# OpenSpaceAI/Nesie

Hardware: AMD Instinct MI355X
Metric: ScanNet scenes/sec (fwd+bwd, 40k pts, bs=8) (higher is better)
Workload: dtype f32; 1 GPU; Nesie-VoteNet supervised pretrain step (nesie-votenet-scannet-pretrain-10%): fwd+bwd+AdamW, 40000 pts/scene, fp32, random-init weights; scenes_per_gpu=8, global_batch=8, parallelism=single, world_size=1, hip_graph=True, deterministic_backward=True, index_chain_pipelined=True, forward_cu_budget=232, forward_cu_budget_from_the_head_on=248, grad_allreduce_bytes=10561936, resident_input_scenes=0

## Files before the change

include/nesie_ops.h:

```cpp
#ifndef NESIE_OPS_H_
#define NESIE_OPS_H_

#include <stddef.h>
#include <stdint.h>

#ifdef __cplusplus
extern "C" {
#endif

typedef enum {
  NESIE_OK = 0,
  NESIE_ERR_INVALID_ARG = 1,
  NESIE_ERR_UNSUPPORTED = 2,
  NESIE_ERR_LAUNCH = 3
} nesie_status;

int nesie_abi_version(void);
const char *nesie_last_error(void);

int nesie_set_distance_form(int form);
int nesie_get_distance_form(void);
int nesie_set_cu_count(int n);
int nesie_get_cu_count(void);

// ... 5 lines not shown
                                     int *idx, void *workspace, size_t workspace_bytes,
                                     void *stream);

int nesie_furthest_point_sampling_with_dist_wrapper(int b, int n, int m,
                                                    const float *dist,
                                                    float *temp, int *idx,
                                                    void *stream);

int nesie_ball_query_wrapper(int b, int n, int m, float min_radius,
                             float max_radius, int nsample,
                             const float *new_xyz, const float *xyz, int *idx,
                             void *stream);

int nesie_fps_leaves_index(int b, int n);
int nesie_ball_query_indexed(int b, int n, int m, float min_radius, float max_radius,
                             int nsample, const float *new_xyz, const void *fps_workspace,
                             size_t workspace_bytes, int *idx, void *stream);

int nesie_knn_wrapper(int b, int n, int m, int nsample, const float *xyz,
                      const float *new_xyz, int *idx, float *dist2, void *stream);

int nesie_group_points_forward(int b, int c, int n, int npoints, int nsample,
                               const float *points, const int *idx, float *out,
                               void *stream);

int nesie_group_points_backward(int b, int c, int n, int npoints, int nsample,
                                const float *grad_out, const int *idx,
                                float *grad_points, void *stream);

int nesie_query_and_group_forward(int b, int c, int n, int npoints, int nsample,
                                  const float *xyz, const float *centres,
                                  const float *features, const int *idx, float radius,
                                  float *out, void *stream);
int nesie_query_and_group_backward(int b, int c, int n, int npoints, int nsample,
                                   const float *grad_out, const int *idx, float *grad_features,
                                   void *stream);
int nesie_inverted_index(int b, int n, long long e_total, const int *idx, int *order,
                         int *sources, int *scratch, void *stream);
int nesie_group_points_backward_csr(int b, int c, int n, int npoints, int nsample,
                                    const float *grad_out, const int *order, const int *sources,
                                    float *grad_points, void *stream);
int nesie_query_and_group_backward_csr(int b, int c, int n, int npoints, int nsample,
                                       const float *grad_out, const int *order,
                                       const int *sources, float *grad_features, void *stream);

int nesie_vote_finish_forward(int b, int c, int n, int normalise, const float *raw,
                              const float *seed_points, const float *seed_feats, float *vote_points,
                              float *vote_feats, float *inv_norm, void *stream);
int nesie_vote_finish_backward(int b, int c, int n, int normalise, const float *g_feats,
                               const float *g_points, const float *vote_feats, const float *inv_norm,
                               float *d_raw, void *stream);

int nesie_gather_rows3(int b, int n, int m, const float *xyz, const int *sample, float *centres,
                       void *stream);
int nesie_query_and_group_backward_xyz(int b, int c, int n, int npoints, int nsample, float radius,
                                       const float *grad_out, const int *order,
                                       const int *sources, const int *sample,
                                       const float *d_centres, float *d_xyz, void *stream);

int nesie_three_interpolate_grad_csr(int b, int c, int n, int m, const float *grad_out,
                                     long long grad_out_bstride, const float *weight, const int *order,
                                     const int *sources, float *grad_points, void *stream);

int nesie_gather_points_wrapper(int b, int c, int n, int npoints,
                                const float *points, const int *idx, float *out,
                                void *stream);

int nesie_gather_points_grad_wrapper(int b, int c, int n, int npoints,
                                     const float *grad_out, const int *idx,
                                     float *grad_points, void *stream);

int nesie_three_nn_wrapper(int b, int n, int m, const float *unknown,
                           const float *known, float *dist2, int *idx,
                           void *stream);

int nesie_three_interpolate_wrapper(int b, int c, int m, int n,
                                    const float *points, const int *idx,
                                    const float *weight, float *out,
                                    void *stream);

int nesie_grid_taps(int b, int kprop, int gp, int m, const float *centre, const float *size,
                    const float *heading, const float *mult, const float *plane,
                    const float *known, int *idx, float *weight, float *rel, void *stream);

int nesie_blend_conv_forward(int b, int c, int m, int n, const float *table, int pitch,
                             int seg_off, const int *idx, const float *weight,
                             const float *rel, const float *wx, float *out, int segs,
                             int seg_len, int c_total, int c_offset,
                             float *stat_partial , void *stream);
int nesie_blend_conv_runs(int n, int segs);
int nesie_blend_conv_backward(int b, int c, int m, int n, const float *dy, int pitch, int seg_off, const int *idx, const float *weight,
                              const float *rel, float *d_table, float *d_wx, int segs,
                              int seg_len, void *stream);
int nesie_blend_conv_backward_bn(int b, int c, int m, int n, const float *da, const float *z,
                                 const float *bnb, int pitch, int seg_off, const int *idx,
                                 const float *weight, const float *rel, float *d_table,
                                 float *d_wx, int segs, int seg_len, void *stream);

size_t nesie_blend_conv_backward_workspace_bytes(int b, int c, int n, int segs);
int nesie_blend_conv_backward_staged(int b, int c, int m, int n, const float *dy, const float *z,
                                     const float *bnb, int pitch, int seg_off, const int *idx,
                                     const float *weight, const float *rel, float *d_table,
                                     float *d_wx, int segs, int seg_len, void *workspace,
                                     size_t workspace_bytes, void *stream);
size_t nesie_blend_conv_backward_any_workspace_bytes(int b, int c, int m, int n, int segs);
int nesie_blend_conv_backward_any(int b, int c, int m, int n, const float *dy, const float *z,
                                  const float *bnb, int pitch, int seg_off, const int *idx,
                                  const float *weight, const float *rel, float *d_table,
                                  float *d_wx, int segs, int seg_len, void *workspace,
                                  size_t workspace_bytes, void *stream);
int nesie_channel_sum(int nb, int ng, int c, long long p, const float *x, long long x_bstride,
                      float *out, void *stream);

int nesie_pw_bnb_coef(int channels, int nslots, double count, const float *part,
                      const float *z_coef, const float *gamma, float *bnb, float *dgamma,
                      float *dbeta, void *stream);

int nesie_three_interpolate_grad_wrapper(int b, int c, int n, int m,
                                         const float *grad_out, const int *idx,
                                         const float *weight,
                                         float *grad_points, void *stream);

int nesie_sort_vertices_forward(int b, int n, int m, const float *vertices,
                                const uint8_t *mask, const int *num_valid,
                                int *idx, void *stream);

int nesie_points_in_boxes_batch(int b, int boxes_num, int pts_num,
                                const float *boxes, const float *pts, int *out,
                                void *stream);

int nesie_points_in_boxes_gpu(int b, int boxes_num, int pts_num, const float *boxes,
                              const float *pts, int *out, void *stream);

int nesie_roiaware_pool3d_sizes(int boxes_num, int pts_num, int channels, int out_x, int out_y,
                                int out_z, int max_pts_each_voxel, long long *out);
int nesie_roiaware_pool3d_forward(int boxes_num, int pts_num, int channels,
                                  int max_pts_each_voxel, int out_x, int out_y, int out_z,
                                  const float *rois, const float *pts, const float *pts_feature,
                                  int *argmax, int *pts_idx_of_voxels, float *pooled_features,
                                  int *pts_voxel, int pool_method, void *stream);
int nesie_roiaware_pool3d_backward(int boxes_num, int pts_num, int out_x, int out_y, int out_z,
                                   int channels, int max_pts_each_voxel,
                                   const int *pts_idx_of_voxels, const int *argmax,
                                   const int *pts_voxel, const float *grad_out, float *grad_in,
                                   int pool_method, void *stream);

int nesie_group_max_pool_forward(long long rows, int nsample, const float *x, float *out,
                                 uint8_t *argmax, void *stream);
int nesie_group_max_pool_backward(long long rows, int nsample, const float *grad_out,
                                  const uint8_t *argmax, float *grad_x, void *stream);
int nesie_group_max_pool_backward_add(long long rows, int nsample, const float *grad_out,
                                      const uint8_t *argmax, float *grad_x, void *stream);

int nesie_lhs_nms_samecls(int b, int k, const float *boxes, float thr, uint8_t *keep,
                          void *stream);

int nesie_iou3d_forward(int n, const float *box1, const float *box2, float *iou, float *jac,
                        void *stream);

int nesie_giou3d_forward(int n, const float *box1, const float *box2, int kind, int enclosing,
                         float *loss, float *iou, float *jac, void *stream);

int nesie_aa_iou3d_paired_forward(int n, const float *box1, const float *box2, int mode, float eps,
                                  float *out, float *jac1, float *jac2, void *stream);
int nesie_aa_iou3d_matrix_forward(int b, int m, int n, const float *box1, const float *box2,
                                  int mode, float eps, float *out, void *stream);
// ... 222 lines not shown
```

nesie_amd/csrc/interpolate.hip:

```cpp
#include "common.h"
#include <math.h>

namespace nesie {

constexpr int NN_BLOCK = 256;
constexpr int NN_TILE = 1024;

template <int FORM>
__global__ __launch_bounds__(NN_BLOCK) void three_nn_kernel(
    int n, int m, const float *__restrict__ unknown, const float *__restrict__ known,
    float *__restrict__ dist2, int *__restrict__ idx) {
  __shared__ float4 kk[NN_TILE];
  const int bi = blockIdx.y;
  const int q = blockIdx.x * NN_BLOCK + threadIdx.x;
  const bool live = q < n;
  unknown += (size_t)bi * n * 3;
  known += (size_t)bi * m * 3;
  const int qq = live ? q : n - 1;
  const float ux = unknown[qq * 3 + 0], uy = unknown[qq * 3 + 1], uz = unknown[qq * 3 + 2];
  float b1 = INFINITY, b2 = INFINITY, b3 = INFINITY;
  int i1 = 0, i2 = 0, i3 = 0;
  for (int t0 = 0; t0 < m; t0 += NN_TILE) {
    const int tn = m - t0 < NN_TILE ? m - t0 : NN_TILE;
    __syncthreads();
    for (int i = threadIdx.x; i < tn; i += NN_BLOCK)
      kk[i] = make_float4(known[(t0 + i) * 3 + 0], known[(t0 + i) * 3 + 1],
                          known[(t0 + i) * 3 + 2], 0.f);
    __syncthreads();
#pragma unroll 4
    for (int i = 0; i < tn; ++i) {
      const float4 kp = kk[i];
      const float d = sqdist_form<FORM>(ux - kp.x, uy - kp.y, uz - kp.z);
      if (d < b3) {
        const int k = t0 + i;
        if (d < b1) {
          b3 = b2; i3 = i2; b2 = b1; i2 = i1; b1 = d; i1 = k;
        } else if (d < b2) {
          b3 = b2; i3 = i2; b2 = d; i2 = k;
        } else {
          b3 = d; i3 = k;
        }
      }
    }
  }
  if (live) {
    float *od = dist2 + ((size_t)bi * n + q) * 3;
    int *oi = idx + ((size_t)bi * n + q) * 3;
    od[0] = b1; od[1] = b2; od[2] = b3;
    oi[0] = i1; oi[1] = i2; oi[2] = i3;
  }
}

template <int FORM>
__global__ __launch_bounds__(NN_BLOCK) void grid_taps_kernel(
    int kprop, int gp, int m, const float *__restrict__ centre, const float *__restrict__ size,
    const float *__restrict__ heading, const float *__restrict__ mult,
    const float *__restrict__ plane, const float *__restrict__ known, int *__restrict__ idx,
    float *__restrict__ weight, float *__restrict__ rel) {
  __shared__ float4 kk[NN_TILE];
  const int bi = blockIdx.y;
  const int n = kprop * gp;
  const int q = blockIdx.x * NN_BLOCK + threadIdx.x;
  const bool live = q < n;
  const int qq = live ? q : n - 1;
  const int k = qq / gp, g = qq - k * gp;
  const float *c3 = centre + ((size_t)bi * kprop + k) * 3;
  const float *s3 = size + ((size_t)bi * kprop + k) * 3;
  const float cx = c3[0], cy = c3[1], cz = c3[2];
  float l[3];
#pragma unroll
  for (int d = 0; d < 3; ++d) {
    const float f = __fmul_rn(mult[g * 3 + d], s3[d]) / 2.f;
    l[d] = __fadd_rn(f, __fmul_rn(f, plane[g * 3 + d]));
  }
  const float h = heading[(size_t)bi * kprop + k];
  const float ch = cosf(h), sh = sinf(h);
  const float ux = __fadd_rn(__fadd_rn(__fmul_rn(l[0], ch), __fmul_rn(l[1], sh)), cx);
  const float uy = __fadd_rn(__fadd_rn(__fmul_rn(l[0], -sh), __fmul_rn(l[1], ch)), cy);
  const float uz = __fadd_rn(l[2], cz);
  known += (size_t)bi * m * 3;
  float b1 = INFINITY, b2 = INFINITY, b3 = INFINITY;
  int i1 = 0, i2 = 0, i3 = 0;
  for (int t0 = 0; t0 < m; t0 += NN_TILE) {
    const int tn = m - t0 < NN_TILE ? m - t0 : NN_TILE;
    __syncthreads();
    for (int i = threadIdx.x; i < tn; i += NN_BLOCK)
      kk[i] = make_float4(known[(t0 + i) * 3 + 0], known[(t0 + i) * 3 + 1],
                          known[(t0 + i) * 3 + 2], 0.f);
    __syncthreads();
#pragma unroll 4
    for (int i = 0; i < tn; ++i) {
      const float4 kp = kk[i];
      const float d = sqdist_form<FORM>(ux - kp.x, uy - kp.y, uz - kp.z);
      if (d < b3) {
        const int kidx = t0 + i;
        if (d < b1) {
          b3 = b2; i3 = i2; b2 = b1; i2 = i1; b1 = d; i1 = kidx;
        } else if (d < b2) {
          b3 = b2; i3 = i2; b2 = d; i2 = kidx;
        } else {
          b3 = d; i3 = kidx;
        }
      }
    }
  }
  if (live) {
    const size_t o = ((size_t)bi * n + q) * 3;
    const float w1 = 1.f / __fadd_rn(sqrtf(b1), 1e-8f), w2 = 1.f / __fadd_rn(sqrtf(b2), 1e-8f),
                w3 = 1.f / __fadd_rn(sqrtf(b3), 1e-8f);
    const float ws = __fadd_rn(__fadd_rn(w1, w2), w3);
    idx[o] = i1; idx[o + 1] = i2; idx[o + 2] = i3;
    weight[o] = w1 / ws; weight[o + 1] = w2 / ws; weight[o + 2] = w3 / ws;
    rel[o] = ux - cx; rel[o + 1] = uy - cy; rel[o + 2] = uz - cz;
  }
}

constexpr int TI_BLOCK = 256;
constexpr int TI_CH = 8;

__global__ __launch_bounds__(TI_BLOCK) void three_interpolate_kernel(
    int c, int m, int n, const float *__restrict__ points, const int *__restrict__ idx,
    const float *__restrict__ weight, float *__restrict__ out) {
  const int p = blockIdx.x * TI_BLOCK + threadIdx.x;
  const int c0 = blockIdx.y * TI_CH;
  const int bi = blockIdx.z;
  if (p >= n) return;
  const int *ix = idx + ((size_t)bi * n + p) * 3;
  const float *w = weight + ((size_t)bi * n + p) * 3;
  int j0 = ix[0], j1 = ix[1], j2 = ix[2];
  j0 = j0 < 0 ? 0 : (j0 >= m ? m - 1 : j0);
  j1 = j1 < 0 ? 0 : (j1 >= m ? m - 1 : j1);
  j2 = j2 < 0 ? 0 : (j2 >= m ? m - 1 : j2);
  const float w0 = w[0], w1 = w[1], w2 = w[2];
  const int cend = c - c0 < TI_CH ? c - c0 : TI_CH;
#pragma unroll
  for (int i = 0; i < TI_CH; ++i) {
    if (i < cend) {
      const float *src = points + ((size_t)bi * c + c0 + i) * m;
      float r = __fadd_rn(__fadd_rn(__fmul_rn(w0, src[j0]), __fmul_rn(w1, src[j1])),
                          __fmul_rn(w2, src[j2]));
      out[((size_t)bi * c + c0 + i) * n + p] = r;
    }
  }
}

constexpr int TS_Q = 64;
constexpr int BF_LD = TS_Q + 1;
typedef float bf_f2 __attribute__((ext_vector_type(2)));
constexpr int BF_NQ = 8;

template <int CPT, bool WX, bool STAT>
__global__ __launch_bounds__(256) void blend_fwd_kernel(
    int c, int cb, int m, int n, int segs, int seg_len, int c_total, int c_offset, int pitch,
    int seg_off, const float *__restrict__ table, const int *__restrict__ idx,
    const float *__restrict__ weight, const float *__restrict__ rel,
    const float *__restrict__ wx, float *__restrict__ out, float *__restrict__ stat_partial,
    int nb) {
#pragma clang fp contract(off)
  constexpr int CW = CPT * 64;
  extern __shared__ float bf_lds[];
  float *tile = bf_lds;
  float *red = bf_lds + CW * BF_LD;
  const int bi = blockIdx.x % nb;
  const int q0 = (blockIdx.x / nb) * TS_Q;
  const int c0 = cb + blockIdx.y * CW;
  const int per_seg = n / segs;
  const int sg = q0 / per_seg, r0 = q0 - sg * per_seg;
  const int lane = threadIdx.x & 63, wv = threadIdx.x >> 6;
  int pj[3];
  float pw[3], pr[3];
  {
    const int r = r0 + wv * 16 + (lane & 15);
    const int k = r / seg_len, g = r - k * seg_len;
    const size_t p = (size_t)bi * n + (size_t)(k * segs + sg) * seg_len + g;
#pragma unroll
    for (int t = 0; t < 3; ++t) {
      const int j = idx[p * 3 + t];
      pj[t] = j < 0 ? 0 : (j >= m ? m - 1 : j);
      pw[t] = weight[p * 3 + t];
      pr[t] = WX ? rel[p * 3 + t] : 0.f;
    }
  }
  const float *feat = table + (size_t)bi * m * pitch + (size_t)sg * seg_off + c0;
  const unsigned voff = (unsigned)(lane * CPT * 4);
  float x[CPT][3] = {};
  if (WX) {
    __builtin_memcpy(&x[0][0], wx + ((size_t)sg * c + c0 + lane * CPT) * 3, sizeof(x));
  }
  constexpr int CP2 = CPT / 2;
  bf_f2 s2[CP2 ? CP2 : 1], q2[CP2 ? CP2 : 1];
  float s1 = 0.f, q1 = 0.f;
#pragma unroll
  for (int e = 0; e < CP2; ++e) s2[e] = q2[e] = bf_f2{0.f, 0.f};
#pragma unroll
  for (int i0 = 0; i0 < 16; i0 += BF_NQ) {
    float a[BF_NQ][3][CPT];
// ... 414 lines not shown
      int u = 0;
      for (; u + 3 < cntj; u += 4) {
        Row v[4];
#pragma unroll
        for (int k = 0; k < 4; ++k) v[k].load(base + (size_t)__builtin_amdgcn_readlane(myslot, u + k) * C);
#pragma unroll
        for (int k = 0; k < 4; ++k)
#pragma unroll
          for (int e = 0; e < CPT; ++e) acc.v[e] += v[k].v[e];
      }
      for (; u < cntj; ++u) {
        Row v;
        v.load(base + (size_t)__builtin_amdgcn_readlane(myslot, u) * C);
#pragma unroll
        for (int e = 0; e < CPT; ++e) acc.v[e] += v.v[e];
      }
    }
  }
  acc.store(d_table + ((size_t)bi * m + seed) * pitch + (size_t)sg * seg_off + lane * CPT);
}

__global__ __launch_bounds__(TI_BLOCK) void three_interpolate_grad_kernel(
    int c, int n, int m, const float *__restrict__ grad_out, const int *__restrict__ idx,
    const float *__restrict__ weight, float *__restrict__ grad_points) {
  const int p = blockIdx.x * TI_BLOCK + threadIdx.x;
  const int c0 = blockIdx.y * TI_CH;
  const int bi = blockIdx.z;
  if (p >= n) return;
  const int *ix = idx + ((size_t)bi * n + p) * 3;
  const float *w = weight + ((size_t)bi * n + p) * 3;
  int j0 = ix[0], j1 = ix[1], j2 = ix[2];
  j0 = j0 < 0 ? 0 : (j0 >= m ? m - 1 : j0);
  j1 = j1 < 0 ? 0 : (j1 >= m ? m - 1 : j1);
  j2 = j2 < 0 ? 0 : (j2 >= m ? m - 1 : j2);
  const float w0 = w[0], w1 = w[1], w2 = w[2];
  const int cend = c - c0 < TI_CH ? c - c0 : TI_CH;
#pragma unroll
  for (int i = 0; i < TI_CH; ++i) {
    if (i < cend) {
      const float g = grad_out[((size_t)bi * c + c0 + i) * n + p];
      float *dst = grad_points + ((size_t)bi * c + c0 + i) * m;
      atomicAdd(dst + j0, __fmul_rn(g, w0));
      atomicAdd(dst + j1, __fmul_rn(g, w1));
      atomicAdd(dst + j2, __fmul_rn(g, w2));
    }
  }
}

}

using namespace nesie;

extern "C" int nesie_three_nn_wrapper(int b, int n, int m, const float *unknown,
                                      const float *known, float *dist2, int *idx,
                                      void *stream) {
  const char *W = "three_nn_wrapper";
  NESIE_REQUIRE(b >= 0 && n >= 0 && m >= 0, W);
  if (b == 0 || n == 0) return NESIE_OK;
  NESIE_REQUIRE(unknown && dist2 && idx && (m == 0 || known), W);
  NESIE_REQUIRE(b <= 65535 && (long long)n * 3 < (1ll << 31) && (long long)m * 3 < (1ll << 31), W);
#define NN(FORM)                                                                          \
  hipLaunchKernelGGL(three_nn_kernel<FORM>, dim3(cdiv(n, NN_BLOCK), b), dim3(NN_BLOCK), 0, \
                     (hipStream_t)stream, n, m, unknown, known, dist2, idx)
  if (distance_form() == 1) NN(1);
  else if (distance_form() == 2) NN(2);
  else NN(0);
#undef NN
  return check_launch(W);
}

extern "C" int nesie_grid_taps(int b, int kprop, int gp, int m, const float *centre,
                               const float *size, const float *heading, const float *mult,
                               const float *plane, const float *known, int *idx, float *weight,
                               float *rel, void *stream) {
  const char *W = "grid_taps";
  NESIE_REQUIRE(b >= 0 && kprop >= 0 && gp >= 0 && m >= 0, W);
  if (b == 0 || kprop == 0 || gp == 0) return NESIE_OK;
  NESIE_REQUIRE(m >= 3 && centre && size && heading && mult && plane && known, W);
  NESIE_REQUIRE(idx && weight && rel && b <= 65535 && (long long)kprop * gp * 3 < (1ll << 31), W);
#define GT(FORM)                                                                                \
  hipLaunchKernelGGL(grid_taps_kernel<FORM>, dim3(cdiv((long long)kprop * gp, NN_BLOCK), b),     \
                     dim3(NN_BLOCK), 0, (hipStream_t)stream, kprop, gp, m, centre, size, heading, \
                     mult, plane, known, idx, weight, rel)
  if (distance_form() == 1) GT(1);
  else if (distance_form() == 2) GT(2);
  else GT(0);
#undef GT
  return check_launch(W);
}

extern "C" int nesie_three_interpolate_wrapper(int b, int c, int m, int n,
                                               const float *points, const int *idx,
                                               const float *weight, float *out,
                                               void *stream) {
  const char *W = "three_interpolate_wrapper";
  NESIE_REQUIRE(b >= 0 && c >= 0 && m >= 0 && n >= 0, W);
  if (b == 0 || c == 0 || n == 0) return NESIE_OK;
  NESIE_REQUIRE(m >= 1 && points && idx && weight && out, W);
  NESIE_REQUIRE(b <= 65535 && cdiv(c, TI_CH) <= 65535, W);
  hipLaunchKernelGGL(three_interpolate_kernel, dim3(cdiv(n, TI_BLOCK), cdiv(c, TI_CH), b),
                     dim3(TI_BLOCK), 0, (hipStream_t)stream, c, m, n, points, idx, weight,
                     out);
  return check_launch(W);
}

static int blend_check(const char *W, int b, int c, int m, int n, int segs, int seg_len,
                       int pitch, int seg_off) {
  NESIE_REQUIRE(b >= 0 && c >= 0 && m >= 0 && n >= 0 && segs >= 1 && seg_len >= 1, W);
  NESIE_REQUIRE(n % (segs * seg_len) == 0 && seg_off >= 0, W);
  NESIE_REQUIRE(pitch >= (long long)(segs - 1) * seg_off + c, W);
  NESIE_REQUIRE(b <= 65535 && cdiv(c, TI_CH) <= 65535, W);
  return NESIE_OK;
}

template <int CPT>
static void blend_fwd_launch(int chunks, int cb, int b, int c, int m, int n, int segs, int seg_len,
                             int c_total, int c_offset, int pitch, int seg_off, const float *table,
                             const int *idx, const float *weight, const float *rel, const float *wx,
                             float *out, float *stat_partial, hipStream_t s) {
  if (chunks <= 0) return;
  constexpr int CW = CPT * 64;
  const size_t lds = (size_t)CW * (BF_LD + 4 * 2) * sizeof(float);
  const dim3 grid((unsigned)((n / TS_Q) * b), (unsigned)chunks);
#define BF(WXF, STF)                                                                              \
  do {                                                                                            \
    static bool attr = false;                                                                     \
    if (!attr) {                                                                                  \
      (void)hipFuncSetAttribute((const void *)blend_fwd_kernel<CPT, WXF, STF>,                    \
                                hipFuncAttributeMaxDynamicSharedMemorySize, (int)lds);            \
      attr = true;                                                                                \
    }                                                                                             \
    hipLaunchKernelGGL((blend_fwd_kernel<CPT, WXF, STF>), grid, dim3(256), lds, s, c, cb, m, n,   \
                       segs, seg_len, c_total, c_offset, pitch, seg_off, table, idx, weight, rel, \
                       wx, out, stat_partial, b);                                                 \
  } while (0)
  if (wx) { if (stat_partial) BF(true, true); else BF(true, false); }
  else { if (stat_partial) BF(false, true); else BF(false, false); }
#undef BF
}

extern "C" int nesie_blend_conv_forward(int b, int c, int m, int n, const float *table,
                                        int pitch, int seg_off, const int *idx,
                                        const float *weight, const float *rel, const float *wx,
                                        float *out, int segs, int seg_len, int c_total,
                                        int c_offset, float *stat_partial, void *stream) {
  const char *W = "blend_conv_forward";
  int st = blend_check(W, b, c, m, n, segs, seg_len, pitch, seg_off);
  if (st) return st;
  NESIE_REQUIRE(c_offset >= 0 && c_offset + c <= c_total && (wx == nullptr) == (rel == nullptr), W);
  if (b == 0 || c == 0 || n == 0) return NESIE_OK;
  NESIE_REQUIRE(m >= 1 && table && idx && weight && out, W);
  if (stat_partial && !(c % 64 == 0 && (n / segs) % TS_Q == 0)) {
    set_error("%s: stat_partial needs c %% 64 == 0 and %d-multiple faces", W, TS_Q);
    return NESIE_ERR_UNSUPPORTED;
  }
  if (c % 64 == 0 && (n / segs) % TS_Q == 0) {
    NESIE_REQUIRE((long long)(n / TS_Q) * b < (1ll << 31) && ((uintptr_t)out & 15) == 0, W);
    blend_fwd_launch<4>(c / 256, 0, b, c, m, n, segs, seg_len, c_total, c_offset, pitch, seg_off, table,
                        idx, weight, rel, wx, out, stat_partial, (hipStream_t)stream);
    const int cb = c / 256 * 256, left = (c - cb) / 64;
#define REST(N) blend_fwd_launch<N>(1, cb, b, c, m, n, segs, seg_len, c_total, c_offset, pitch, seg_off, table, \
                                    idx, weight, rel, wx, out, stat_partial, (hipStream_t)stream)
    if (left == 1) REST(1); else if (left == 2) REST(2); else if (left == 3) REST(3);
#undef REST
  } else
    hipLaunchKernelGGL(blend_fwd_generic_kernel, dim3(cdiv(n, TI_BLOCK), cdiv(c, TI_CH), b),
// ... 144 lines not shown
```

nesie_amd/kernels.py:

```python
import contextlib
import os

import ctypes

import torch

from . import _lib

_injected = None


def _no_cpu_path(device):
    return RuntimeError(
        "nesie_amd kernels need HIP device tensors (got device "
        f"{device}); there is no CPU path in the product")


def _check(*tensors):
    for t in tensors:
        if not t.is_cuda:
            raise _no_cpu_path(t.device)
        if not t.is_contiguous():
            raise RuntimeError("nesie_amd kernels need contiguous tensors")

# ... 301 lines not shown

    def affine_relu_maxpool_forward(self, x, coef, pooled, argmax):
        _check(x, coef, pooled, argmax); _f32(x, coef, pooled)
        b, c, m, ns = x.shape
        assert tuple(coef.shape) == (c, 4) and tuple(pooled.shape) == (b, c, m)
        assert argmax.dtype == torch.uint8 and tuple(argmax.shape) == (b, c, m)
        _launch("nesie_affine_relu_maxpool_forward", x, b, c, m, ns, x, coef, pooled, argmax)

    def mlp_stream_forward(self, x, w, y, stat_partial=None, in_coef=None, in_relu=False):
        _check(x, w); _f32(x, w)
        b, cin, p = x.shape
        cout = w.shape[0]
        assert tuple(w.shape) == (cout, cin)
        if y is not None:
            _check(y); _f32(y)
            assert tuple(y.shape) == (b, cout, p)
        else:
            assert stat_partial is not None
        if stat_partial is not None:
            _check(stat_partial); _f32(stat_partial)
            assert tuple(stat_partial.shape) == (self.mlp_stream_parts(b, p), cout, 2)
        _launch("nesie_mlp_layer_forward_stream", x, b, cin, cout, p, x, cin * p, w, in_coef,
                bool(in_relu), y, stat_partial)

    @staticmethod
    def mlp_stream_parts(b, p):
        return int(_lib.load().nesie_mlp_stream_partials(b, p))

    def aligned_3d_nms(self, boxes, scores, classes, valid, thr, picks, count):
        _check(boxes, scores, classes, picks, count); _f32(boxes, scores); _i32(classes, picks, count)
        b, k = scores.shape
        assert tuple(boxes.shape) == (b, k, 6) and tuple(classes.shape) == (b, k)
        assert tuple(picks.shape) == (b, k) and count.numel() == b
        if valid is not None:
            _check(valid)
            assert valid.dtype == torch.uint8 and tuple(valid.shape) == (b, k)
        _launch("nesie_aligned_3d_nms", boxes, b, k, boxes, scores, classes, valid, float(thr),
                picks, count)

    def points_in_boxes_count(self, boxes, pts, counts):
        _check(boxes, pts, counts); _f32(boxes, pts); _i32(counts)
        b, t, _ = boxes.shape
        assert pts.shape[0] == b and pts.shape[2] == 3 and tuple(counts.shape) == (b, t)
        _launch("nesie_points_in_boxes_count", boxes, b, t, pts.shape[1], boxes, pts, counts)

    def boxes_overlap_bev(self, boxes_a, boxes_b, ans_overlap):
        _check(boxes_a, boxes_b, ans_overlap); _f32(boxes_a, boxes_b, ans_overlap)
        n, m = boxes_a.shape[0], boxes_b.shape[0]
        assert boxes_a.shape[1] == 5 and boxes_b.shape[1] == 5
        assert tuple(ans_overlap.shape) == (n, m)
        _launch("nesie_boxes_overlap_bev", boxes_a, n, boxes_a, m, boxes_b, ans_overlap)

    def bev_nms(self, boxes, scores, valid, offsets, max_seg, thr, rotated, keep, count, ws):
        _check(boxes, scores, offsets, keep, count, ws); _f32(boxes, scores); _i32(offsets, keep, count)
        n, s = scores.numel(), count.numel()
        assert tuple(boxes.shape) == (n, 5) and offsets.numel() == s + 1 and keep.numel() == n
        if valid is not None:
            _check(valid)
            assert valid.dtype == torch.uint8 and valid.numel() == n
        _launch("nesie_bev_nms", boxes, n, s, int(max_seg), boxes, scores, valid, offsets,
                float(thr), 1 if rotated else 0, keep, count, ws, ws.numel() * ws.element_size())

    def scene_assemble(self, pool, height, choices, xform, out):
        _check(pool, height, choices, xform, out); _f32(pool, height, xform, out); _i32(choices)
        b, n = choices.shape
        assert pool.dim() == 2 and pool.shape[1] == 3 and height.numel() == pool.shape[0]
        assert tuple(xform.shape) == (b, 20) and tuple(out.shape) == (b, n, 4)
        _launch("nesie_scene_assemble", pool, b, n, pool.shape[0], pool, height, choices, xform,
                out)

    def grid_taps(self, centre, size, heading, mult, plane, known):
        _check(centre, size, heading, mult, plane, known)
        _f32(centre, size, heading, mult, plane, known)
        b, k = centre.shape[:2]
        gp, m = mult.shape[0], known.shape[1]
        assert tuple(size.shape) == (b, k, 3) and tuple(heading.shape) == (b, k)
        assert tuple(plane.shape) == (gp, 3) and known.shape[0] == b
        idx = torch.empty(b, k * gp, 3, dtype=torch.int32, device=centre.device)
        weight = torch.empty(b, k * gp, 3, dtype=torch.float32, device=centre.device)
        rel = torch.empty_like(weight)
        _launch("nesie_grid_taps", centre, b, k, gp, m, centre, size, heading, mult, plane, known,
                idx, weight, rel)
        return idx, weight, rel

    def blend_conv_forward(self, table, seg_off, idx, weight, rel, wx, out, segs, seg_len,
                           c, c_offset, stat_partial=None):
        _check(table, idx, weight, out); _f32(table, weight, out); _i32(idx)
        b, m, pitch = table.shape
        n = idx.shape[1]
        assert idx.numel() == b * n * 3 and weight.numel() == b * n * 3
        assert n % (segs * seg_len) == 0 and out.dim() == 4
        assert out.shape[0] == b and out.shape[1] == segs and out.shape[3] * segs == n
        assert c_offset + c <= out.shape[2] and (rel is None) == (wx is None)
        if wx is not None:
            _check(rel, wx); _f32(rel, wx)
            assert rel.numel() == b * n * 3 and tuple(wx.shape) == (segs, c, 3)
        if stat_partial is not None:
            _check(stat_partial); _f32(stat_partial)
            assert stat_partial.numel() == segs * c * (b * (n // segs // 64)) * 2
        _launch("nesie_blend_conv_forward", table, b, c, m, n, table, pitch, seg_off, idx, weight,
                rel, wx, out, segs, seg_len, int(out.shape[2]), c_offset, stat_partial)

    DETERMINISTIC = os.environ.get('NESIE_DETERMINISTIC', '1') != '0'

    @classmethod
    def set_deterministic(cls, on=True):
        prev, cls.DETERMINISTIC = cls.DETERMINISTIC, bool(on)
        return prev

    def scatter_index(self, idx, n):
        if not self.DETERMINISTIC:
            return None
        return self.inverted_index(idx.contiguous(), n)

    def blend_backward_writes_table(self, c, n, segs, m):
        return blend_backward_form(c, n // segs, m, self.DETERMINISTIC) != 'atomic'

    def blend_conv_backward(self, dy, seg_off, idx, weight, rel, d_table, d_wx, segs, seg_len,
                            bn_z=None, bnb=None):
        _check(dy, idx, weight, d_table); _f32(dy, weight, d_table); _i32(idx)
        b, m, pitch = d_table.shape
        n, c = idx.shape[1], dy.shape[2]
        assert tuple(dy.shape) == (b, segs, c, n // segs)
        if d_wx is not None:
            _check(rel, d_wx); _f32(rel, d_wx)
            assert tuple(d_wx.shape) == (segs, c, 3)
        if bnb is not None:
            _check(bn_z, bnb); _f32(bn_z, bnb)
            assert tuple(bn_z.shape) == tuple(dy.shape) and tuple(bnb.shape) == (segs * c, 8)
        form = blend_backward_form(c, n // segs, m, self.DETERMINISTIC)
        if form == 'any':
            self.blend_conv_backward_any(dy, seg_off, idx, weight, rel, d_table, d_wx, segs, seg_len,
                                         bn_z=bn_z, bnb=bnb)
            return
        part = None
        if d_wx is not None:
            runs = _lib.load().nesie_blend_conv_runs(n, segs)
            part = torch.empty(b * runs, segs, c, 3, dtype=torch.float32, device=dy.device)
        if form == 'staged':
            assert seg_off == c or segs == 1, 'staged form: one column block per face'
            need = _lib.load().nesie_blend_conv_backward_workspace_bytes(b, c, n, segs)
            ws = torch.empty(need, dtype=torch.uint8, device=dy.device)
            _launch("nesie_blend_conv_backward_staged", dy, b, c, m, n, dy, bn_z, bnb, pitch,
                    seg_off, idx, weight, rel, d_table, part, segs, seg_len, ws, need)
        elif bnb is not None:
            _launch("nesie_blend_conv_backward_bn", dy, b, c, m, n, dy, bn_z, bnb, pitch, seg_off,
                    idx, weight, rel, d_table, part, segs, seg_len)
        else:
            _launch("nesie_blend_conv_backward", dy, b, c, m, n, dy, pitch, seg_off, idx, weight,
                    rel, d_table, part, segs, seg_len)
        if part is not None:
            torch.sum(part, 0, out=d_wx)

    def blend_conv_backward_any(self, dy, seg_off, idx, weight, rel, d_table, d_wx, segs, seg_len,
                                bn_z=None, bnb=None):
        _check(dy, idx, weight, d_table); _f32(dy, weight, d_table); _i32(idx)
        b, m, pitch = d_table.shape
        n, c = idx.shape[1], dy.shape[2]
        assert tuple(dy.shape) == (b, segs, c, n // segs)
        if pitch != (segs - 1) * seg_off + c or not (seg_off == c or segs == 1):
            d_table.zero_()
        need = _lib.load().nesie_blend_conv_backward_any_workspace_bytes(b, c, m, n, segs)
        ws = _workspace(need, dy.device)
        _launch("nesie_blend_conv_backward_any", dy, b, c, m, n, dy, bn_z, bnb, pitch, seg_off, idx,
                weight, rel, d_table, d_wx, segs, seg_len, ws, need)

# ... 925 lines not shown
```

nesie_amd/votenet/side_pooling.py:

```python
import numpy as np
import torch
import torch.nn as nn

from .. import grad_slots
from ..kernels import backend_for
from ..mmdet3d_ops import blend_conv, three_interpolate_segmented, three_nn
from ..mmdet3d_ops.pool import group_max_pool, group_max_pool_shared
from ..mmdet3d_ops.norm import FusedBNReLU1d, FusedBNReLU2d
from ..mmdet3d_ops.pointnet_modules import PointwiseConv1d, PointwiseConv2d, pointwise_conv


def rot_gpu(t):
    c, s = torch.cos(t), torch.sin(t)
    z, o = torch.zeros_like(t), torch.ones_like(t)
    return torch.stack([torch.stack([c, s, z], -1), torch.stack([-s, c, z], -1),
                        torch.stack([z, z, o], -1)], -2)


class _TableProduct(torch.autograd.Function):

    @staticmethod
    def forward(ctx, features, w):
        ctx.save_for_backward(features, w)
        return torch.matmul(features, w.t())
# ... 251 lines not shown
    B, S = x.shape[:2]
    convs = [layers for layers in zip(*heads) if isinstance(layers[0], PointwiseConv1d)]
    groups = [[l.weight.flatten(1) for l in layers] for layers in convs] \
        + [[l.bias for l in layers] for layers in convs if layers[0].bias is not None]
    stacked = iter(fused_mlp.stack_groups(groups))
    weights = {id(layers[0]): next(stacked) for layers in convs}
    biases = {id(layers[0]): next(stacked) for layers in convs if layers[0].bias is not None}
    steps = [layers for layers in zip(*heads) if not isinstance(layers[0], nn.Identity)]
    fused = _heads_as_stack(heads, x, steps, weights, biases)
    if fused is not None:
        return fused
    held = None
    for i, layers in enumerate(steps):
        first = layers[0]
        if isinstance(first, PointwiseConv1d):
            x = torch.matmul(weights[id(first)].unsqueeze(0), x)
            if first.bias is not None:
                if i + 1 < len(steps) and isinstance(steps[i + 1][0], FusedBNReLU1d):
                    held = biases[id(first)].reshape(-1)
                else:
                    x = x + biases[id(first)].view(1, S, -1, 1)
        elif isinstance(first, FusedBNReLU1d):
            C, P = x.shape[2], x.shape[3]
            x = _stacked_bn(layers, x.reshape(B, S * C, P), row_bias=held).view(B, S, C, P)
            held = None
        else:
            raise TypeError(f'batched_heads: unsupported layer {type(first).__name__}')
    return x


def _heads_as_stack(heads, x, steps, weights, biases):
    from ..mmdet3d_ops import fused_mlp
    B, S, cin, P = x.shape
    convs, norms = [], []
    i = 0
    while i < len(steps):
        if not isinstance(steps[i][0], PointwiseConv1d):
            return None
        convs.append(steps[i])
        if i + 1 < len(steps) and isinstance(steps[i + 1][0], FusedBNReLU1d):
            norms.append(steps[i + 1])
            i += 2
        else:
            norms.append(None)
            i += 1
    shapes = [(c[0].in_channels, c[0].out_channels) for c in convs]
    if not fused_mlp.stack1d_supported(backend_for(x), x.reshape(B * S, cin, P), shapes,
                                       [None if n is None else n[0] for n in norms], S):
        return None
    bn_groups = [g for n in norms if n is not None for g in ([l.weight for l in n], [l.bias for l in n])]
    stacked = iter(fused_mlp.stack_groups(bn_groups)) if bn_groups else iter(())
    gammas, betas, stats = [], [], []
    for n in norms:
        if n is None:
            gammas.append(None); betas.append(None); stats.append(None)
        else:
            gammas.append(grad_slots.reshaped(next(stacked), -1))
            betas.append(grad_slots.reshaped(next(stacked), -1))
            pack = stacked_running_stats(list(n))
            stats.append((pack[0], pack[1]))
    w = [weights[id(c[0])] for c in convs]
    b = [grad_slots.reshaped(biases[id(c[0])], -1) if c[0].bias is not None else None for c in convs]
    y = fused_mlp.stack1d(x.reshape(B * S, cin, P), [list(c) for c in convs],
                          [None if n is None else list(n) for n in norms], S=S, weights=w, biases=b,
                          gammas=gammas, betas=betas, stats=stats)
    return y.view(B, S, y.shape[1], P)


def heads_batchable(heads, x):
    if backend_for(x).name != 'hip' or x.dtype != torch.float32:
        return False
    for layers in zip(*heads):
        t = type(layers[0])
        if any(type(l) is not t for l in layers):
            return False
        if isinstance(layers[0], FusedBNReLU1d):
            if not _stackable_bn(layers):
                return False
        elif not isinstance(layers[0], (PointwiseConv1d, nn.Identity)):
            return False
    return True


def _score_head(in_ch, out_ch):
    return nn.Sequential(PointwiseConv1d(in_ch, 128, 1), FusedBNReLU1d(128), nn.Identity(),
                         PointwiseConv1d(128, 128, 1), FusedBNReLU1d(128), nn.Identity(),
                         PointwiseConv1d(128, out_ch, 1))


class SidePooling(nn.Module):
    grid_size = 4
    hide_dim = 256
    plane_axes = None

    def __init__(self, num_class, num_heading_bin, num_size_cluster, mean_size_arr_path,
                 num_proposal, sampling, seed_feat_dim=256, query_feats='seed',
                 iou_class_depend=True):
        super().__init__()
        self.num_class = num_class
        self.num_heading_bin = num_heading_bin
        self.num_size_cluster = num_size_cluster
        self.mean_size_arr = None
        self.num_proposal = num_proposal
        self.sampling = sampling
        self.seed_feat_dim = seed_feat_dim
        self.query_feats = query_feats
        self.iou_class_depend = iou_class_depend
        self.reg_topk = 4
        g = self.grid_size
        self.left_mask = [i // g * g * g + i % g for i in range(g * g)]
        self.right_mask = [i // g * g * g + i % g + g * (g - 1) for i in range(g * g)]
        face_idx = (list(range(0, g * g)) + list(range(g ** 3 - g * g, g ** 3))
                    + list(range(g - 1, g ** 3, g)) + list(range(0, g ** 3, g))
                    + self.left_mask + self.right_mask)
        self.register_buffer('_face_idx', torch.tensor(face_idx, dtype=torch.long),
                             persistent=False)
        plane = None
        if self.plane_axes is not None:
            plane = torch.zeros(6, 3)
            for f, a in enumerate(self.plane_axes):
                plane[f, a] = 0.1
            self.register_buffer('_plane_axis', plane, persistent=False)
        self._register_grid_tables(face_idx, plane)
        self.iou_size = num_class if iou_class_depend else 1
        before, head = [], []
        for _ in range(6):
            before.append(MiniPointNet(seed_feat_dim + 3, 128, hide_dim=self.hide_dim))
            head.append(self._side_head(128 + 33 + 4 + 1))
        self._add_final(before, head)
        self.mlps_before = nn.ModuleList(before)
        self.mlps_head = nn.ModuleList(head)

    def _side_head(self, in_ch):
        return _score_head(in_ch, self.iou_size)

    def _add_final(self, before, head):
        before.append(MiniPointNet(self.seed_feat_dim + 3, 128, hide_dim=self.hide_dim))
        head.append(_score_head(128, self.iou_size))

    def stacked_parameter_groups(self):
        groups = []
        for modules in (list(self.mlps_before[:6]), list(self.mlps_head[:6])):
            per = [list(m.parameters()) for m in modules]
            if len(per) == 6 and all(len(p) == len(per[0]) for p in per):
                groups += [list(kind) for kind in zip(*per)
                           if all(t.shape == kind[0].shape for t in kind)]
        return groups

    def _register_grid_tables(self, face_idx, plane=None):
        g = self.grid_size
        step = torch.linspace(-1, 1, g)
        full = torch.stack([step.view(g, 1, 1).expand(g, g, g), step.view(1, g, 1).expand(g, g, g),
                            step.view(1, 1, g).expand(g, g, g)], -1).reshape(-1, 3)
        side = full[torch.tensor(face_idx)]
        if plane is not None:
            g2 = g * g
            side = side.view(6, g2, 3)
            pl = plane.view(6, 1, 3).expand(6, g2, 3)
            side, plane = (torch.cat([side, side, side], 1).reshape(-1, 3),
                           torch.cat([-pl, torch.zeros_like(pl), pl], 1).reshape(-1, 3))
        else:
            plane = torch.zeros_like(side)
        self.register_buffer('_mult_box', full.contiguous(), persistent=False)
        self.register_buffer('_mult_side', side.contiguous(), persistent=False)
        self.register_buffer('_plane_side', plane.contiguous(), persistent=False)

    def fused_taps(self, origin_xyz, center, size, heading, which):
        mult = self._mult_side if which == 'side' else self._mult_box
        plane = self._plane_side if which == 'side' else torch.zeros_like(mult)
        return backend_for(origin_xyz).grid_taps(center.contiguous(), size.contiguous(),
                                                 heading.contiguous(), mult, plane, origin_xyz)

    def extract_features(self, end_points):
        return (end_points['seed_points'].detach().contiguous(),
                end_points['seed_features'].detach().transpose(1, 2).contiguous())

    def generate_grid(self, size):
        B, K = size.shape[:2]
        g = self.grid_size
        step = torch.linspace(-1, 1, g, device=size.device)
        gx = step.view(g, 1, 1).repeat(1, g, g).view(1, 1, -1).expand(B, K, -1)
        gy = step.view(1, g, 1).repeat(g, 1, g).view(1, 1, -1).expand(B, K, -1)
        gz = step.view(1, 1, g).repeat(g, g, 1).view(1, 1, -1).expand(B, K, -1)
        x_grid = gx * size[:, :, 0:1] / 2
        y_grid = gy * size[:, :, 1:2] / 2
        z_grid = gz * size[:, :, 2:3] / 2
        return torch.cat([x_grid.unsqueeze(-1), y_grid.unsqueeze(-1), z_grid.unsqueeze(-1)],
                         dim=-1)

    def _to_scene(self, grid, center, heading):
        B, K = center.shape[:2]
        rot_mat = rot_gpu(heading).view(-1, 3, 3)
        grid = torch.bmm(grid.reshape(B * K, -1, 3), rot_mat.transpose(1, 2)).view(B, K, -1, 3)
        return grid + center.unsqueeze(2)

    def grid_for_side(self, whole_grid, center, heading):
        side_grid = torch.index_select(whole_grid, 2, self._face_idx)
        return self._to_scene(side_grid, center, heading)

    def grid_for_bbox(self, whole_grid, center, heading):
        return self._to_scene(whole_grid, center, heading)

    def _blend_taps(self, origin_xyz, whole_grid, center):
        B, K = center.shape[:2]
        grid_size = whole_grid.shape[1] // K
        _, idx = three_nn(whole_grid, origin_xyz)
        interp_points = torch.gather(origin_xyz, 1, idx.view(B, -1, 1).expand(-1, -1, 3).long())
        expanded = whole_grid.unsqueeze(2).expand(-1, -1, 3, -1).reshape(B, -1, 3)
        dist = interp_points - expanded
        dist = torch.sqrt(torch.sum(dist * dist, dim=2))
        relative_grid = whole_grid - center.unsqueeze(2).expand(-1, -1, grid_size, -1) \
            .reshape(B, -1, 3)
        weight = (1 / (dist + 1e-8)).view(B, -1, 3)
        weight = (weight / torch.sum(weight, dim=2, keepdim=True)).contiguous()
        return idx, weight, relative_grid.contiguous()

    def first_conv_through_blend(self, nets, origin_xyz, origin_features, whole_grid, center,
                                 taps=None):
        K = center.shape[1]
        segs = len(nets)
        idx, weight, rel = taps if taps is not None \
            else self._blend_taps(origin_xyz, whole_grid, center)
        G = idx.shape[1] // (K * segs)
        from ..mmdet3d_ops import fused_mlp
        w = fused_mlp.stack_groups([[net.first_conv[0].weight.flatten(1) for net in nets]])[0]
        w_xyz, w_feat = fused_mlp.SplitXyzFeat.apply(w)
        table = _TableProduct.apply(origin_features, w_feat)
        return DeferredBlendConv(table, w_xyz, idx, weight, rel, segs, G, K)

    def grid_features(self, origin_xyz, origin_features, whole_grid, center, segs=1):
        B, K = center.shape[:2]
        grid_size = whole_grid.shape[1] // K
        idx, weight, relative_grid = self._blend_taps(origin_xyz, whole_grid, center)
        G, C = grid_size // segs, origin_features.shape[2]
        out = origin_features.new_empty(B, segs, 3 + C, K * G)
        out[:, :, :3] = relative_grid.view(B, K, segs, G, 3).permute(0, 2, 4, 1, 3) \
            .reshape(B, segs, 3, K * G)
        three_interpolate_segmented(origin_features, idx, weight, out, segs, G, 3)
        return out.view(B, segs, 3 + C, K, G)

    def dist_feature(self, end_points, prefix='', copies=2):
        prob = end_points[f'{prefix}bbox_probs'].detach()
        backend = backend_for(prob)
        if (backend.name == 'hip' and self.reg_topk == 4 and prob.dtype == torch.float32
                and prob.dim() == 4 and prob.shape[1] == 6 and prob.shape[2] >= 5):
            return backend.side_prob_stats(prob.contiguous(), copies)
        stat = torch.cat([prob, prob.topk(self.reg_topk, dim=2)[0],
                          prob.var(dim=2, keepdim=True)], dim=2)
        return stat.permute(1, 0, 2, 3).repeat(1, 1, 1, copies)

    def _side_input(self, center, size, heading, end_points, prefix):
        B, K = size.shape[:2]
        origin_xyz, origin_features = self.extract_features(end_points)
        nets, box_net = list(self.mlps_before[:6]), self.mlps_before[6:7]
        box_in = None
        fused = backend_for(origin_xyz).name == 'hip'
        if fused:
            c0 = self.first_conv_through_blend(
                nets, origin_xyz, origin_features, None, center,
                taps=self.fused_taps(origin_xyz, center, size, heading, 'side'))
            if len(box_net):
                box_in = dict(conv0_out=self.first_conv_through_blend(
                    box_net, origin_xyz, origin_features, None, center,
                    taps=self.fused_taps(origin_xyz, center, size, heading, 'box')))
        else:
            whole_grid = self.generate_grid(size)
            side_grid = self.grid_for_side(whole_grid, center, heading).view(B, -1, 3).contiguous()
            side_feats = self.grid_features(origin_xyz, origin_features, side_grid, center, segs=6)
            if len(box_net):
                bbox_grid = self.grid_for_bbox(whole_grid, center, heading).view(B, -1, 3) \
                    .contiguous()
                box_in = dict(points=self.grid_features(origin_xyz, origin_features, bbox_grid,
                                                        center)[:, 0])
        dist_feature = self.dist_feature(end_points, prefix,
                                         copies=K // end_points[f'{prefix}bbox_probs'].shape[-1])
        if fused and mini_pointnets_groupable(nets, c0):
            pooled = grouped_mini_pointnets(nets, c0)
        elif fused:
            c0 = c0.materialize()[0]
            pooled = torch.stack([nets[i](conv0_out=c0[:, i]) for i in range(6)], 1)
        else:
            pooled = torch.stack([nets[i](side_feats[:, i]) for i in range(6)], 1)
        return torch.cat([pooled, dist_feature.transpose(0, 1)], dim=2), box_in

    def _side_scores(self, x):
        heads = list(self.mlps_head[:6])
        if heads_batchable(heads, x[:, 0]):
            return batched_heads(heads, x).transpose(0, 1).contiguous()
        return torch.stack([heads[i](x[:, i]) for i in range(6)], 0)

    def forward(self, center, size, heading, end_points, prefix=''):
        x, box_in = self._side_input(center, size, heading, end_points, prefix)
        end_points[f'{prefix}side_scores'] = self._side_scores(x)
        bbox_feats = self.mlps_before[6](**box_in)
        if heads_batchable([self.mlps_head[6]], bbox_feats):
            iou = batched_heads([self.mlps_head[6]], bbox_feats.unsqueeze(1)).squeeze(1)
        else:
            iou = self.mlps_head[6](bbox_feats)
        end_points[f'{prefix}iou_scores'] = iou.transpose(2, 1)
        return end_points
```

Baseline: 691.7 scenes/s.

## Share grid-tap nearest-neighbour search across side and box grids via deduplicated offsets

Adds a grid_taps_shared kernel that finds the 3 nearest seeds and interpolation weights only once per distinct grid offset (mult, plane) for each proposal. It then scatters the result to every slot in the side and box tap sets that uses that offset. The Python side builds a dedup map at init and prefetches both tap sets in one launch, which fused_taps then consumes. This is meant to remove the repeated O(m) nearest-neighbour scans for grid points that appear in both the side and box grids, and one kernel launch. It adds scatter writes and version-checked caching logic.

```diff
diff --git a/include/nesie_ops.h b/include/nesie_ops.h
--- a/include/nesie_ops.h
+++ b/include/nesie_ops.h
@@ -111,6 +111,12 @@
 int nesie_grid_taps(int b, int kprop, int gp, int m, const float *centre, const float *size,
                     const float *heading, const float *mult, const float *plane,
                     const float *known, int *idx, float *weight, float *rel, void *stream);
+
+int nesie_grid_taps_shared(int b, int kprop, int nd, int m, const float *centre,
+                           const float *size, const float *heading, const float *mult_d,
+                           const float *plane_d, const float *known, const int *slot_ptr,
+                           const int *slot, int gp0, int gp1, int *idx0, float *weight0,
+                           float *rel0, int *idx1, float *weight1, float *rel1, void *stream);
 
 int nesie_blend_conv_forward(int b, int c, int m, int n, const float *table, int pitch,
                              int seg_off, const int *idx, const float *weight,
diff --git a/nesie_amd/csrc/interpolate.hip b/nesie_amd/csrc/interpolate.hip
--- a/nesie_amd/csrc/interpolate.hip
+++ b/nesie_amd/csrc/interpolate.hip
@@ -51,34 +51,39 @@
   }
 }
 
+struct GridTap {
+  float cx, cy, cz;
+  float ux, uy, uz;
+  float b1, b2, b3;
+  int i1, i2, i3;
+};
+
+__device__ __forceinline__ void grid_tap_point(GridTap &t, const float *__restrict__ centre,
+                                               const float *__restrict__ size,
+                                               const float *__restrict__ heading,
+                                               const float *__restrict__ mult,
+                                               const float *__restrict__ plane, size_t prop,
+                                               int row) {
+  const float *c3 = centre + prop * 3;
+  const float *s3 = size + prop * 3;
+  t.cx = c3[0]; t.cy = c3[1]; t.cz = c3[2];
+  float l[3];
+#pragma unroll
+  for (int d = 0; d < 3; ++d) {
+    const float f = __fmul_rn(mult[row * 3 + d], s3[d]) / 2.f;
+    l[d] = __fadd_rn(f, __fmul_rn(f, plane[row * 3 + d]));
+  }
+  const float h = heading[prop];
+  const float ch = cosf(h), sh = sinf(h);
+  t.ux = __fadd_rn(__fadd_rn(__fmul_rn(l[0], ch), __fmul_rn(l[1], sh)), t.cx);
+  t.uy = __fadd_rn(__fadd_rn(__fmul_rn(l[0], -sh), __fmul_rn(l[1], ch)), t.cy);
+  t.uz = __fadd_rn(l[2], t.cz);
+}
+
 template <int FORM>
-__global__ __launch_bounds__(NN_BLOCK) void grid_taps_kernel(
-    int kprop, int gp, int m, const float *__restrict__ centre, const float *__restrict__ size,
-    const float *__restrict__ heading, const float *__restrict__ mult,
-    const float *__restrict__ plane, const float *__restrict__ known, int *__restrict__ idx,
-    float *__restrict__ weight, float *__restrict__ rel) {
-  __shared__ float4 kk[NN_TILE];
-  const int bi = blockIdx.y;
-  const int n = kprop * gp;
-  const int q = blockIdx.x * NN_BLOCK + threadIdx.x;
-  const bool live = q < n;
-  const int qq = live ? q : n - 1;
-  const int k = qq / gp, g = qq - k * gp;
-  const float *c3 = centre + ((size_t)bi * kprop + k) * 3;
-  const float *s3 = size + ((size_t)bi * kprop + k) * 3;
-  const float cx = c3[0], cy = c3[1], cz = c3[2];
-  float l[3];
-#pragma unroll
-  for (int d = 0; d < 3; ++d) {
-    const float f = __fmul_rn(mult[g * 3 + d], s3[d]) / 2.f;
-    l[d] = __fadd_rn(f, __fmul_rn(f, plane[g * 3 + d]));
-  }
-  const float h = heading[(size_t)bi * kprop + k];
-  const float ch = cosf(h), sh = sinf(h);
-  const float ux = __fadd_rn(__fadd_rn(__fmul_rn(l[0], ch), __fmul_rn(l[1], sh)), cx);
-  const float uy = __fadd_rn(__fadd_rn(__fmul_rn(l[0], -sh), __fmul_rn(l[1], ch)), cy);
-  const float uz = __fadd_rn(l[2], cz);
-  known += (size_t)bi * m * 3;
+__device__ __forceinline__ void grid_tap_scan(GridTap &t, float4 *kk,
+                                              const float *__restrict__ known, int m) {
+  const float ux = t.ux, uy = t.uy, uz = t.uz;
   float b1 = INFINITY, b2 = INFINITY, b3 = INFINITY;
   int i1 = 0, i2 = 0, i3 = 0;
   for (int t0 = 0; t0 < m; t0 += NN_TILE) {
@@ -104,14 +109,74 @@
       }
     }
   }
-  if (live) {
-    const size_t o = ((size_t)bi * n + q) * 3;
-    const float w1 = 1.f / __fadd_rn(sqrtf(b1), 1e-8f), w2 = 1.f / __fadd_rn(sqrtf(b2), 1e-8f),
-                w3 = 1.f / __fadd_rn(sqrtf(b3), 1e-8f);
-    const float ws = __fadd_rn(__fadd_rn(w1, w2), w3);
+  t.b1 = b1; t.b2 = b2; t.b3 = b3;
+  t.i1 = i1; t.i2 = i2; t.i3 = i3;
+}
+
+struct GridTapOut {
+  float w1, w2, w3, rx, ry, rz;
+  int i1, i2, i3;
+  __device__ __forceinline__ explicit GridTapOut(const GridTap &t) : i1(t.i1), i2(t.i2), i3(t.i3) {
+    const float v1 = 1.f / __fadd_rn(sqrtf(t.b1), 1e-8f), v2 = 1.f / __fadd_rn(sqrtf(t.b2), 1e-8f),
+                v3 = 1.f / __fadd_rn(sqrtf(t.b3), 1e-8f);
+    const float ws = __fadd_rn(__fadd_rn(v1, v2), v3);
+    w1 = v1 / ws; w2 = v2 / ws; w3 = v3 / ws;
+    rx = t.ux - t.cx; ry = t.uy - t.cy; rz = t.uz - t.cz;
+  }
+  __device__ __forceinline__ void store(int *__restrict__ idx, float *__restrict__ weight,
+                                        float *__restrict__ rel, size_t o) const {
     idx[o] = i1; idx[o + 1] = i2; idx[o + 2] = i3;
-    weight[o] = w1 / ws; weight[o + 1] = w2 / ws; weight[o + 2] = w3 / ws;
-    rel[o] = ux - cx; rel[o + 1] = uy - cy; rel[o + 2] = uz - cz;
+    weight[o] = w1; weight[o + 1] = w2; weight[o + 2] = w3;
+    rel[o] = rx; rel[o + 1] = ry; rel[o + 2] = rz;
+  }
+};
+
+template <int FORM>
+__global__ __launch_bounds__(NN_BLOCK) void grid_taps_kernel(
+    int kprop, int gp, int m, const float *__restrict__ centre, const float *__restrict__ size,
+    const float *__restrict__ heading, const float *__restrict__ mult,
+    const float *__restrict__ plane, const float *__restrict__ known, int *__restrict__ idx,
+    float *__restrict__ weight, float *__restrict__ rel) {
+  __shared__ float4 kk[NN_TILE];
+  const int bi = blockIdx.y;
+  const int n = kprop * gp;
+  const int q = blockIdx.x * NN_BLOCK + threadIdx.x;
+  const bool live = q < n;
+  const int qq = live ? q : n - 1;
+  const int k = qq / gp, g = qq - k * gp;
+  GridTap t;
+  grid_tap_point(t, centre, size, heading, mult, plane, (size_t)bi * kprop + k, g);
+  grid_tap_scan<FORM>(t, kk, known + (size_t)bi * m * 3, m);
+  if (live) GridTapOut(t).store(idx, weight, rel, ((size_t)bi * n + q) * 3);
+}
+
+template <int FORM>
+__global__ __launch_bounds__(NN_BLOCK) void grid_taps_shared_kernel(
+    int kprop, int nd, int m, const float *__restrict__ centre, const float *__restrict__ size,
+    const float *__restrict__ heading, const float *__restrict__ mult_d,
+    const float *__restrict__ plane_d, const float *__restrict__ known,
+    const int *__restrict__ slot_ptr, const int *__restrict__ slot, int gp0, int gp1,
+    int *__restrict__ idx0, float *__restrict__ weight0, float *__restrict__ rel0,
+    int *__restrict__ idx1, float *__restrict__ weight1, float *__restrict__ rel1) {
+  __shared__ float4 kk[NN_TILE];
+  const int bi = blockIdx.y;
+  const int n = kprop * nd;
+  const int q = blockIdx.x * NN_BLOCK + threadIdx.x;
+  const bool live = q < n;
+  const int qq = live ? q : n - 1;
+  const int k = qq / nd, d = qq - k * nd;
+  const size_t prop = (size_t)bi * kprop + k;
+  GridTap t;
+  grid_tap_point(t, centre, size, heading, mult_d, plane_d, prop, d);
+  grid_tap_scan<FORM>(t, kk, known + (size_t)bi * m * 3, m);
+  if (!live) return;
+  const GridTapOut out(t);
+  const int nslot = gp0 + gp1;
+  const int lo = max(slot_ptr[d], 0), hi = min(slot_ptr[d + 1], nslot);
+  for (int j = lo; j < hi; ++j) {
+    const int s = slot[j];
+    if (s >= 0 && s < gp0) out.store(idx0, weight0, rel0, (prop * gp0 + s) * 3);
+    else if (s >= gp0 && s < nslot) out.store(idx1, weight1, rel1, (prop * gp1 + (s - gp0)) * 3);
   }
 }
 
@@ -692,6 +757,37 @@
   hipLaunchKernelGGL(grid_taps_kernel<FORM>, dim3(cdiv((long long)kprop * gp, NN_BLOCK), b),     \
                      dim3(NN_BLOCK), 0, (hipStream_t)stream, kprop, gp, m, centre, size, heading, \
                      mult, plane, known, idx, weight, rel)
+  if (distance_form() == 1) GT(1);
+  else if (distance_form() == 2) GT(2);
+  else GT(0);
+#undef GT
+  return check_launch(W);
+}
+
+extern "C" int nesie_grid_taps_shared(int b, int kprop, int nd, int m, const float *centre,
+                                      const float *size, const float *heading,
+                                      const float *mult_d, const float *plane_d,
+                                      const float *known, const int *slot_ptr, const int *slot,
+                                      int gp0, int gp1, int *idx0, float *weight0, float *rel0,
+                                      int *idx1, float *weight1, float *rel1, void *stream) {
+  const char *W = "grid_taps_shared";
+  NESIE_REQUIRE(b >= 0 && kprop >= 0 && nd >= 0 && m >= 0 && gp0 >= 0 && gp1 >= 0, W);
+  if (b == 0 || kprop == 0 || gp0 + (long long)gp1 == 0) return NESIE_OK;
+  NESIE_REQUIRE(gp0 >= 1 && nd >= 1 && nd <= gp0 + (long long)gp1, W);
+  NESIE_REQUIRE(m >= 3 && centre && size && heading && mult_d && plane_d && known, W);
+  NESIE_REQUIRE(slot_ptr && slot && idx0 && weight0 && rel0, W);
+  NESIE_REQUIRE(gp1 == 0 || (idx1 && weight1 && rel1), W);
+  if (b > 65535 || (long long)kprop * (gp0 > gp1 ? gp0 : gp1) * 3 >= (1ll << 31) ||
+      gp0 + (long long)gp1 >= (1ll << 31)) {
+    set_error("%s: b = %d scenes or %d proposals of %d + %d grid points are more than the "
+              "kernel indexes", W, b, kprop, gp0, gp1);
+    return NESIE_ERR_UNSUPPORTED;
+  }
+#define GT(FORM)                                                                                  \
+  hipLaunchKernelGGL(grid_taps_shared_kernel<FORM>, dim3(cdiv((long long)kprop * nd, NN_BLOCK), b), \
+                     dim3(NN_BLOCK), 0, (hipStream_t)stream, kprop, nd, m, centre, size, heading,   \
+                     mult_d, plane_d, known, slot_ptr, slot, gp0, gp1, idx0, weight0, rel0, idx1,   \
+                     weight1, rel1)
   if (distance_form() == 1) GT(1);
   else if (distance_form() == 2) GT(2);
   else GT(0);
diff --git a/nesie_amd/kernels.py b/nesie_amd/kernels.py
--- a/nesie_amd/kernels.py
+++ b/nesie_amd/kernels.py
@@ -407,6 +407,27 @@
         _launch("nesie_grid_taps", centre, b, k, gp, m, centre, size, heading, mult, plane, known,
                 idx, weight, rel)
         return idx, weight, rel
+
+    def grid_taps_shared(self, centre, size, heading, mult_d, plane_d, slot_ptr, slot, gps, known):
+        _check(centre, size, heading, mult_d, plane_d, slot_ptr, slot, known)
+        _f32(centre, size, heading, mult_d, plane_d, known); _i32(slot_ptr, slot)
+        b, k = centre.shape[:2]
+        nd, m = mult_d.shape[0], known.shape[1]
+        gps = tuple(int(g) for g in gps)
+        assert len(gps) in (1, 2) and min(gps) >= 1
+        assert tuple(size.shape) == (b, k, 3) and tuple(heading.shape) == (b, k)
+        assert tuple(mult_d.shape) == (nd, 3) and tuple(plane_d.shape) == (nd, 3)
+        assert slot_ptr.numel() == nd + 1 and slot.numel() == sum(gps) and known.shape[0] == b
+        out = []
+        for gp in gps:
+            idx = torch.empty(b, k * gp, 3, dtype=torch.int32, device=centre.device)
+            weight = torch.empty(b, k * gp, 3, dtype=torch.float32, device=centre.device)
+            out.append((idx, weight, torch.empty_like(weight)))
+        second = out[1] if len(gps) == 2 else (None, None, None)
+        _launch("nesie_grid_taps_shared", centre, b, k, nd, m, centre, size, heading, mult_d,
+                plane_d, known, slot_ptr, slot, gps[0], gps[1] if len(gps) == 2 else 0,
+                *out[0], *second)
+        return out
 
     def blend_conv_forward(self, table, seg_off, idx, weight, rel, wx, out, segs, seg_len,
                            c, c_offset, stat_partial=None):
diff --git a/nesie_amd/votenet/side_pooling.py b/nesie_amd/votenet/side_pooling.py
--- a/nesie_amd/votenet/side_pooling.py
+++ b/nesie_amd/votenet/side_pooling.py
@@ -357,6 +357,38 @@
     return True
 
 
+def shared_tap_map(sets, lead=0):
+    bits = [torch.cat([m, p], 1).to(torch.float32).contiguous().view(torch.int32) for m, p in sets]
+    start = [0]
+    for b in bits:
+        start.append(start[-1] + b.shape[0])
+    number, row = {}, [0] * start[-1]
+    for s in [lead] + [i for i in range(len(sets)) if i != lead]:
+        for g, key in enumerate(map(tuple, bits[s].tolist())):
+            row[start[s] + g] = number.setdefault(key, len(number))
+    served = [[] for _ in number]
+    for slot, d in enumerate(row):
+        served[d].append(slot)
+    ptr = [0]
+    for s in served:
+        ptr.append(ptr[-1] + len(s))
+    distinct = torch.tensor(list(number), dtype=torch.int32).view(-1, 6)
+    return dict(mult=distinct[:, :3].contiguous(), plane=distinct[:, 3:].contiguous(),
+                ptr=torch.tensor(ptr, dtype=torch.int32),
+                slot=torch.tensor([s for group in served for s in group], dtype=torch.int32),
+                row=torch.tensor(row, dtype=torch.long), gps=tuple(b.shape[0] for b in bits))
+
+
+class _ReadyTaps:
+
+    def __init__(self, inputs, sets):
+        self.inputs, self.versions, self.sets = inputs, [t._version for t in inputs], sets
+
+    def serves(self, inputs, which):
+        return which in self.sets and all(
+            a is b and a._version == v for a, b, v in zip(inputs, self.inputs, self.versions))
+
+
 def _score_head(in_ch, out_ch):
     return nn.Sequential(PointwiseConv1d(in_ch, 128, 1), FusedBNReLU1d(128), nn.Identity(),
                          PointwiseConv1d(128, 128, 1), FusedBNReLU1d(128), nn.Identity(),
@@ -405,6 +437,17 @@
         self._add_final(before, head)
         self.mlps_before = nn.ModuleList(before)
         self.mlps_head = nn.ModuleList(head)
+        self._register_tap_map()
+
+    def _register_tap_map(self):
+        self._tap_sets = ('side', 'box') if len(self.mlps_before) > 6 else ('side',)
+        sets = [(self._mult_side, self._plane_side)]
+        if 'box' in self._tap_sets:
+            sets.append((self._mult_box, torch.zeros_like(self._mult_box)))
+        tap_map = shared_tap_map(sets, lead=len(sets) - 1)
+        self._tap_gps = tap_map['gps']
+        for name in ('mult', 'plane', 'ptr', 'slot'):
+            self.register_buffer('_tap_' + name, tap_map[name], persistent=False)
 
     def _side_head(self, in_ch):
         return _score_head(in_ch, self.iou_size)
@@ -440,7 +483,23 @@
         self.register_buffer('_mult_side', side.contiguous(), persistent=False)
         self.register_buffer('_plane_side', plane.contiguous(), persistent=False)
 
+    _taps_ready = None
+
+    def _prefetch_taps(self, origin_xyz, center, size, heading):
+        as_float = lambda bits: bits.view(torch.float32)
+        taps = backend_for(origin_xyz).grid_taps_shared(
+            center.contiguous(), size.contiguous(), heading.contiguous(), as_float(self._tap_mult),
+            as_float(self._tap_plane), self._tap_ptr, self._tap_slot, self._tap_gps, origin_xyz)
+        self._taps_ready = _ReadyTaps((origin_xyz, center, size, heading),
+                                      dict(zip(self._tap_sets, taps)))
+
     def fused_taps(self, origin_xyz, center, size, heading, which):
+        ready, self._taps_ready = self._taps_ready, None
+        if ready is not None and ready.serves((origin_xyz, center, size, heading), which):
+            taps = ready.sets.pop(which)
+            if ready.sets:
+                self._taps_ready = ready
+            return taps
         mult = self._mult_side if which == 'side' else self._mult_box
         plane = self._plane_side if which == 'side' else torch.zeros_like(mult)
         return backend_for(origin_xyz).grid_taps(center.contiguous(), size.contiguous(),
@@ -531,6 +590,7 @@
         box_in = None
         fused = backend_for(origin_xyz).name == 'hip'
         if fused:
+            self._prefetch_taps(origin_xyz, center, size, heading)
             c0 = self.first_conv_through_blend(
                 nets, origin_xyz, origin_features, None, center,
                 taps=self.fused_taps(origin_xyz, center, size, heading, 'side'))
```

After: 696.0 scenes/s (median of 6 runs). Within noise of the previous version (+0.6%).
